# tanmud/video_style_transfer

Hardware: AMD Instinct MI355X
Metric: denoised frames/sec, 16x512x512 clip, 50-step AnimateDiff-XL (higher is better)
Workload: dtype bf16; 1 GPU; BASELINE configs[2]: 16x512x512 clip + UnZipLoRA rank-8 (fused) on all 560 spatial q/k/v/out, 50-step Euler, CFG 7.5 batched (B=2); model=SDXL UNet + AnimateDiff-SDXL motion modules (synthetic weights), global_batch=1, frames=16, resolution=512, parallelism=single, graph=True

## Files before the change

include/vst.h:

```cpp
#ifndef VST_H
#define VST_H
#include <stddef.h>
#ifdef __cplusplus
extern "C" {
#endif

int vst_gemm(const void* A, int lda, const void* A2, int lda2, int K1, const void* W, int ldw, int M, int N, int K,
             const float* bias, const float* row_bias, int row_bias_div, int ld_row_bias, const void* R, int ldr,
             void* C, int ldc, int epilogue, void* stream);
int vst_gemm_ex(const void* A, int lda, const void* A2, int lda2, int K1, const void* W, int ldw, int M, int N, int K,
                const float* bias, const float* row_bias, int row_bias_div, int ld_row_bias, const void* R, int ldr,
                void* C, int ldc, int epilogue, int tile, int splits, void* workspace, size_t ws_bytes,
                void* stream);
size_t vst_gemm_workspace_bytes(int M, int N, int K);

int vst_gemm_lora(const void* x, int ldx, const void* Acat, int ld_acat, int P, int group_n, int group_r,
                  const void* W, int ldw, int M, int N, int K, const float* bias, const void* R, int ldr,
                  void* C, int ldc, void* stream);
int vst_gemm_lora_supported(int M, int N, int K, int P, int group_n, int group_r);
int vst_p8_force_bn(int bn);
int vst_p8_conv(int on);
int vst_p8_persist(int on);

int vst_gemm_temporal_attention(const void* x, int ldx, const void* Wt, int ldw, const float* bias, int M, int K,
                                int nclip, int F, int HW, int heads, int head_dim, float scale, void* O, int ldo,
                                void* stream);
int vst_gemm_temporal_attention_supported(int M, int K, int nclip, int F, int HW, int heads, int head_dim);

int vst_gemm_cross_attention(const void* x, int ldx, const void* Acat, int ld_acat, int P, int group_n, int group_r,
                             const void* W, int ldw, const float* bias, int M, int N, int K, const void* Kt,
                             const void* Vt, int ldkv, int nkv_rows, int Nq, int Nk, int kv_div, float scale, void* O,
                             int ldo, void* stream);
int vst_gemm_cross_attention_supported(int M, int N, int K, int lora, int P, int group_n, int group_r, int Nq,
                                       int Nk);

const char* vst_gemm_kernel_name(int M, int N, int K, int kind, int tile, int splits, size_t ws_bytes);

int vst_conv3x3(const void* x1, int C1, const void* x2, int C2, int nimg, int H, int W, int stride, int upsample,
                const void* Wt, int Cout, const float* bias, const float* row_bias, int row_bias_div, const void* R,
                int ldr, void* out, int ldc, void* stream);
int vst_conv3x3_ex(const void* x1, int C1, const void* x2, int C2, int nimg, int H, int W, int stride, int upsample,
                   const void* Wt, int Cout, const float* bias, const float* row_bias, int row_bias_div,
                   int ld_row_bias, const void* R, int ldr, void* out, int ldc, int tile, int splits, void* workspace,
                   size_t ws_bytes, void* stream);
int vst_conv3x3_colstat(const void* x1, int C1, const void* x2, int C2, int nimg, int H, int W, int stride,
                        int upsample, const void* Wt, int Cout, const float* bias, const float* row_bias,
                        int row_bias_div, int ld_row_bias, const void* R, int ldr, void* out, int ldc,
                        float* colstat, void* stream);

int vst_spatial_attention(const void* q, int ldq, const void* k, const void* v, int ldkv, void* o, int ldo,
                          int nbatch, int heads, int Nq, int Nk, int kv_div, int head_dim, float scale, float* lse,
                          void* stream);
int vst_sa_self(int on);

int vst_temporal_attention(const void* q, const void* k, const void* v, int ldqkv, void* o, int ldo, int nclip,
                           int F, int HW, int heads, int head_dim, float scale, void* stream);

int vst_temporal_attention_windowed(const void* q, const void* k, const void* v, int ldqkv, const float* pos_q,
                                    const float* pos_k, const float* pos_v, int ldpos, void* o, int ldo, int nclip,
                                    int F, int HW, int heads, int head_dim, int L, int S, int weighting, float scale,
                                    void* stream);

int vst_motion_attention_block(const void* x, int ldx, int nclip, int F, int HW, int C, int heads, const float* gamma,
                               const float* beta, float eps, const float* pe, const void* wqkv, int ldw,
                               const float* bqkv, const void* wo, int ldwo, const float* bo, float scale, void* y,
                               int ldy, void* stream);
int vst_motion_attention_block_supported(int C, int F, int HW, int heads);

size_t vst_groupnorm_workspace_bytes(int nsamples, int rows_per_sample, int groups, int C);
int vst_groupnorm(const void* x1, int ld1, int C1, const void* x2, int ld2, int C2, int nsamples,
                  int rows_per_sample, int groups, float eps, const float* gamma, const float* beta, int silu_act,
                  void* y, int ldy, void* workspace, void* stream);
int vst_colstat(const void* x, int ldx, int M, int C, float* cs, void* stream);
int vst_groupnorm_colstat(const void* x1, int ld1, int C1, const float* cs1, const void* x2, int ld2, int C2,
                          const float* cs2, int nsamples, int rows_per_sample, int groups, float eps,
// ... 88 lines not shown
```

video_style_transfer_amd/_lib.py:

```python
from __future__ import annotations

import ctypes
import os

_HERE = os.path.dirname(os.path.abspath(__file__))
LIB_PATH = os.path.join(_HERE, "libvst_hip.so")

_P = ctypes.c_void_p
_I = ctypes.c_int
_F = ctypes.c_float
_S = ctypes.c_size_t
SIGNATURES = {
    "vst_gemm": (_I, [_P, _I, _P, _I, _I, _P, _I, _I, _I, _I, _P, _P, _I, _I, _P, _I, _P, _I, _I, _P]),
    "vst_gemm_ex": (_I, [_P, _I, _P, _I, _I, _P, _I, _I, _I, _I, _P, _P, _I, _I, _P, _I, _P, _I, _I, _I, _I, _P, _S,
                         _P]),
    "vst_gemm_workspace_bytes": (_S, [_I, _I, _I]),
    "vst_gemm_lora": (_I, [_P, _I, _P, _I, _I, _I, _I, _P, _I, _I, _I, _I, _P, _P, _I, _P, _I, _P]),
    "vst_gemm_lora_supported": (_I, [_I, _I, _I, _I, _I, _I]),
    "vst_gemm_cross_attention": (_I, [_P, _I, _P, _I, _I, _I, _I, _P, _I, _P, _I, _I, _I, _P, _P, _I, _I, _I, _I, _I,
                                      _F, _P, _I, _P]),
    "vst_gemm_cross_attention_supported": (_I, [_I, _I, _I, _I, _I, _I, _I, _I, _I]),
    "vst_gemm_temporal_attention": (_I, [_P, _I, _P, _I, _P, _I, _I, _I, _I, _I, _I, _I, _F, _P, _I, _P]),
    "vst_gemm_temporal_attention_supported": (_I, [_I, _I, _I, _I, _I, _I, _I]),
    "vst_gemm_kernel_name": (ctypes.c_char_p, [_I, _I, _I, _I, _I, _I, _S]),
    "vst_conv3x3": (_I, [_P, _I, _P, _I, _I, _I, _I, _I, _I, _P, _I, _P, _P, _I, _P, _I, _P, _I, _P]),
    "vst_conv3x3_ex": (_I, [_P, _I, _P, _I, _I, _I, _I, _I, _I, _P, _I, _P, _P, _I, _I, _P, _I, _P, _I, _I, _I, _P,
                            _S, _P]),
    "vst_spatial_attention": (_I, [_P, _I, _P, _P, _I, _P, _I, _I, _I, _I, _I, _I, _I, _F, _P, _P]),
    "vst_temporal_attention": (_I, [_P, _P, _P, _I, _P, _I, _I, _I, _I, _I, _I, _F, _P]),
    "vst_temporal_attention_windowed": (_I, [_P, _P, _P, _I, _P, _P, _P, _I, _P, _I, _I, _I, _I, _I, _I, _I, _I, _I, _F,
                                             _P]),
    "vst_motion_attention_block": (_I, [_P, _I, _I, _I, _I, _I, _I, _P, _P, _F, _P, _P, _I, _P, _P, _I, _P, _F, _P, _I,
                                        _P]),
    "vst_motion_attention_block_supported": (_I, [_I, _I, _I, _I]),
    "vst_groupnorm_workspace_bytes": (_S, [_I, _I, _I, _I]),
    "vst_groupnorm_frame_chunks": (_I, [_I]),
    "vst_p8_force_bn": (_I, [_I]),
    "vst_p8_conv": (_I, [_I]),
    "vst_p8_persist": (_I, [_I]),
    "vst_sa_self": (_I, [_I]),
    "vst_groupnorm_frame_partials": (_I, [_P, _I, _I, _I, _I, _I, _P, _P]),
    "vst_groupnorm_apply_partials": (_I, [_P, _I, _I, _I, _I, _I, _I, _P, _I, _F, _P, _P, _I, _P, _I, _P, _P]),
    "vst_permute_rows": (_I, [_P, _P, _I, _I, _I, _I, _I, _I, _I, _I, _I, _P]),
    "vst_groupnorm": (_I, [_P, _I, _I, _P, _I, _I, _I, _I, _I, _F, _P, _P, _I, _P, _I, _P, _P]),
    "vst_colstat": (_I, [_P, _I, _I, _I, _P, _P]),
    "vst_groupnorm_colstat": (_I, [_P, _I, _I, _P, _P, _I, _I, _P, _I, _I, _I, _F, _P, _P, _I, _P, _I, _P, _P]),
    "vst_conv3x3_colstat": (_I, [_P, _I, _P, _I, _I, _I, _I, _I, _I, _P, _I, _P, _P, _I, _I, _P, _I, _P, _I, _P,
                                 _P]),
    "vst_layernorm_lora": (_I, [_P, _I, _I, _I, _P, _P, _F, _P, _I, _P, _I, _P, _I, _P]),
    "vst_layernorm": (_I, [_P, _I, _I, _I, _P, _P, _F, _P, _I, _I, _P, _I, _P]),
    "vst_add_row_table": (_I, [_P, _I, _I, _I, _P, _I, _I, _P, _I, _P]),
    "vst_unpack_tokens": (_I, [_P, _I, _I, _I, _I, _P, _P]),
    "vst_timestep_embedding": (_I, [_P, _P, _I, _I, _I, _F, _P, _I, _I, _I, _P]),
    "vst_pack_latents": (_I, [_P, _I, _I, _I, _I, _P, _P, _F, _I, _P, _P]),
    "vst_euler_cfg_step": (_I, [_P, _I, _F, _P, _I, _I, _I, _I, _P, _P, _P]),
    "vst_step_advance": (_I, [_P, _I, _P]),
    "vst_silu": (_I, [_P, _P, _S, _P]),
    "vst_add": (_I, [_P, _P, _P, _S, _P]),
    "vst_quick_gelu": (_I, [_P, _P, _S, _P]),
    "vst_embed_tokens": (_I, [_P, _I, _I, _P, _P, _I, _P, _I, _P]),
    "vst_causal_attention": (_I, [_P, _I, _P, _P, _I, _P, _I, _I, _I, _I, _I, _F, _P]),
    "vst_residual_layernorm": (_I, [_P, _I, _P, _I, _I, _I, _P, _P, _F, _P, _I, _P, _I, _P]),
    "vst_copy2d": (_I, [_P, _I, _P, _I, _I, _I, _P]),
    "vst_transpose": (_I, [_P, _I, _I, _I, _P, _I, _P]),
    "vst_layernorm_bwd_workspace_bytes": (_S, [_I, _I]),
    "vst_layernorm_bwd": (_I, [_P, _I, _P, _I, _I, _I, _P, _F, _P, _I, _P, _P, _P, _P]),
    "vst_geglu_bwd": (_I, [_P, _I, _P, _I, _I, _I, _P, _I, _P]),
    "vst_colsum_workspace_bytes": (_S, [_I, _I]),
    "vst_colsum": (_I, [_P, _I, _I, _I, _P, _P, _P]),
    "vst_groupnorm_bwd_workspace_bytes": (_S, [_I, _I, _I, _I]),
    "vst_groupnorm_bwd": (_I, [_P, _I, _P, _I, _I, _I, _I, _I, _F, _P, _P, _I, _P, _I, _P, _P, _P, _P]),
    "vst_spatial_attention_bwd_workspace_bytes": (_S, [_I, _I, _I, _I]),
    "vst_spatial_attention_bwd": (_I, [_P, _I, _P, _P, _I, _P, _I, _P, _I, _P, _P, _I, _P, _P, _I, _I, _I, _I, _I, _I,
                                       _I, _F, _P, _P]),
    "vst_zero_insert": (_I, [_P, _I, _I, _I, _I, _P, _P]),
    "vst_sumpool2x2": (_I, [_P, _I, _I, _I, _I, _P, _P]),
    "vst_temporal_attention_bwd": (_I, [_P, _P, _P, _I, _P, _I, _P, _P, _P, _I, _I, _I, _I, _I, _I, _F, _P]),
    "vst_conv3x3_down_pad0": (_I, [_P, _I, _I, _I, _I, _P, _I, _P, _P, _I, _P, _S, _P]),
    "vst_gemm_f32out": (_I, [_P, _I, _P, _I, _I, _I, _I, _P, _P]),
    "vst_gemm_tn": (_I, [_P, _I, _P, _I, _I, _I, _I, _P, _I, _P, _S, _P]),
    "vst_gemm_tn_workspace_bytes": (_S, [_I, _I, _I]),
    "vst_softmax_rows": (_I, [_P, _I, _I, _I, _F, _P, _I, _P]),
    "vst_nchw_to_nhwc": (_I, [_P, _I, _I, _I, _F, _P, _I, _P]),
    "vst_nhwc_to_nchw": (_I, [_P, _I, _I, _I, _I, _P, _P]),
    "vst_frames_to_u8": (_I, [_P, _I, _I, _I, _I, _P, _P]),
    "vst_vae_sample": (_I, [_P, _I, _I, _I, _P, _F, _P, _P]),
    "vst_probe_mfma": (_I, [_I, _I, _P, _P]),
    "vst_probe_hbm_read": (_I, [_P, _S, _I, _P, _P]),
    "vst_probe_fetch": (_I, [_I, _P, _I, _I, _I, _P, _P]),
    "vst_probe_mix": (_I, [_I, _I, _P, _I, _I, _I, _P, _P]),
    "vst_version": (ctypes.c_char_p, []),
}
# ... 38 lines not shown
```

video_style_transfer_amd/csrc/gemm_common.h:

```cpp
#pragma once
#include "vst_common.h"

namespace vst {

struct GemmArgs {
  const bf16_t* A1; const bf16_t* A2;
  int lda1, lda2, K1;
  int H, W, C1, C2, OH, OW, stride, up;
  int pad0;
  const bf16_t* Wt; int ldw;
  int M, N, K;
  const float* bias;
  const float* rbias; int rbias_div, ldrb;
  const bf16_t* R; int ldr;
  bf16_t* C; int ldc;
  float* ws;
  int splits;
  int act;
  int persist;
  int group_m;
  int p8_bn;
  int ablate;
  uint32_t a1_bytes, a2_bytes, w_bytes, r_bytes;
  const bf16_t* la;
  int lda_la, la_p, la_gn, la_gr;
  uint32_t la_bytes, wtail_bytes;
  const bf16_t* xa_k;
  const bf16_t* xa_v;
  int xa_ldkv, xa_nk, xa_nq, xa_kvdiv;
  float xa_scale_log2;
  uint32_t xa_kv_bytes;
  int ta_hw, ta_heads, ta_d;
  float ta_scale_log2;
  float* colstat;
};

__device__ __forceinline__ int swz(int row, int chunk) {
  return row * 128 + ((chunk ^ ((row >> 1) & 7)) << 4);
}

}
```

video_style_transfer_amd/csrc/gemm_p8.hip:

```cpp
#include "attn_common.h"
#include "gemm_common.h"
#include "gemm_epilogue.h"

#include <type_traits>

namespace vst {

template <int BN_, int BM_ = 256>
struct P8Cfg {
  static constexpr int BM = BM_, BN = BN_, WAVES_M = 2, WAVES_N = 4, NWAVES = 8, THREADS = 512;
  static constexpr int WM = BM / 2, WN = BN / 4, MI = WM / 16, NJ = WN / 16;
  static constexpr int HALF = WM / 2;
  static constexpr int MQR = HALF / 16;
  static constexpr int NPA = BM / 128;
  static constexpr int RB1 = WN - 32;
  static constexpr int NJ1 = RB1 / 16;
  static constexpr int NPB1 = 4 * RB1 / 64;
  static constexpr int SLOT_A = BM / 2 * 128;
  static constexpr int SLOT_B0 = 128 * 128;
  static constexpr int SLOT_B1 = 4 * RB1 * 128;
  static constexpr int BUF = 2 * SLOT_A + SLOT_B0 + SLOT_B1;
  static constexpr int EPI_BYTES = BM * (BN * 2 + 16);
  static constexpr int LDS = 2 * BUF > EPI_BYTES ? 2 * BUF : EPI_BYTES;
  static constexpr int LORA_OFF = 2 * BUF, V_OFF = 2 * BUF + 5 * 1024, LORA_END = V_OFF + BN * 32;
// ... 425 lines not shown
    float ls = 0.f;
#pragma unroll
    for (int i = 0; i < 4; ++i) {
      s[i] = fast_exp2(s[i] * sl2 - mb);
      ls += s[i];
    }
    ls += __shfl_xor(ls, 16);
    ls += __shfl_xor(ls, 32);
    const float inv = 1.0f / ls;
    const u32x2 pw{pack2bf(s[0], s[1]), pack2bf(s[2], s[3])};
    const s16x4 pb = __builtin_bit_cast(s16x4, pw);
    bf16_t* orow = p.C + (size_t)((b * TF + fr) * p.ta_hw + pg * 16 + pl) * p.ldc + h * TD;
    for (int db = 0; db < DB; ++db) {
      const int d = db * 16 + fr;
      s16x4 va = s16x4{0, 0, 0, 0};
      if (d < TD) {
#pragma unroll
        for (int i = 0; i < 4; ++i) va[i] = *reinterpret_cast<const short*>(R + (4 * g + i) * LROW + (cv + d) * 2);
      }
      const f32x4 o = __builtin_amdgcn_mfma_f32_16x16x16bf16_1k(va, pb, f32x4{0.f, 0.f, 0.f, 0.f}, 0, 0, 0) * inv;
      if (db * 16 + 4 * g < TD)
        *reinterpret_cast<u32x2*>(orow + db * 16 + 4 * g) = u32x2{pack2bf(o[0], o[1]), pack2bf(o[2], o[3])};
    }
  }
}

template <int EPI, int BN, bool LORA = false, int PH = 3, int BM = 256, bool CONV = false, bool PERSIST = false>
__global__ __launch_bounds__(512, 1) void gemm_p8_kernel(GemmArgs p) {
  extern __shared__ __attribute__((aligned(16))) char smem[];
  using Cfg = P8Cfg<BN, BM>;
  static_assert(!CONV || (!LORA && EPI == 0), "conv: plain epilogue");
  static_assert(EPI != 1 || BN == 256, "GEGLU needs 64-column [hidden | gate] blocks");
  static_assert(!LORA || EPI != 1, "in-GEMM LoRA: linear epilogue");
  static_assert(!PERSIST || (!CONV && EPI != 4 && EPI != 5 && PH == 2 && (!LORA || (EPI == 0 && BN == 320))),
                "persistent tiles: plain / GEGLU / GELU, and the in-GEMM LoRA on 128x320 tiles; PH 2");
  static_assert(!(PERSIST && LORA) || Cfg::U_END <= 160 * 1024, "LoRA persistent LDS");
  static_assert(EPI != 5 || (BN == 256 && BM == 256 && !LORA && !CONV), "temporal attention epilogue: 256x256 tiles");
  static_assert(EPI != 4 || (BN == 192 && BM == 256), "cross-attention epilogue: 256 x 192 tiles (3 heads)");
#define VST_P8_VMWAIT_LX(X)                  \
  do {                                       \
    if (LORA && wid < 2) p8_vmwait<(X) + 1>(); \
    else p8_vmwait<(X)>();                   \
  } while (0)
  constexpr bool ONE_A = PERSIST || LORA || EPI == 4 || EPI == 5;
#if defined(VST_P8_DMM)
  constexpr bool DMM = true;
#else
  constexpr bool DMM = false;
#endif
#ifdef VST_P8_LORA_B1E
  constexpr bool B1E = EPI != 1;
#else
  constexpr bool B1E = EPI != 1 && !LORA;
#endif
  constexpr int BUF = Cfg::BUF, RB1 = Cfg::RB1, NJ1 = Cfg::NJ1, NPB1 = Cfg::NPB1, NPA = Cfg::NPA;
  constexpr int HALF = Cfg::HALF, MQR = Cfg::MQR;
  auto slot_off = [](int s_) { return s_ < 2 ? s_ * Cfg::SLOT_A : (s_ == 2 ? 2 * Cfg::SLOT_A : 2 * Cfg::SLOT_A + Cfg::SLOT_B0); };
  const int tid = threadIdx.x, lane = tid & 63;
  const int wid = __builtin_amdgcn_readfirstlane(tid >> 6);
  const int wr = wid >> 2, wc = wid & 3;
  const int fr = lane & 15, fq = lane >> 4;
  const int nbm = (p.M + BM - 1) / BM, nbn = (p.N + BN - 1) / BN;
  const int ntiles = nbm * nbn;
  const int GROUP_M = p.group_m > 0 ? p.group_m : 8;
  auto tile_origin = [&](int t, int& m0, int& n0) {
    const int in_group = GROUP_M * nbn;
    const int gid = t / in_group, first_m = gid * GROUP_M;
    const int gsize = min(nbm - first_m, GROUP_M);
    m0 = (first_m + (t - gid * in_group) % gsize) * BM;
    n0 = ((t - gid * in_group) / gsize) * BN;
  };
  const auto ra1 = make_rsrc(p.A1, p.a1_bytes);
  const auto ra2 = make_rsrc(p.A2 ? p.A2 : p.A1, p.A2 ? p.a2_bytes : 0u);
  const auto rw = make_rsrc(p.Wt, p.w_bytes);
  const int nk = (p.K + 63) / 64;
  const bool ktail = !PERSIST && (p.K & 63) != 0;
  const bool late = wid >= 4;
#ifdef VST_P8_TRACE
  const int abl = p.ablate;
#else
  constexpr int abl = 0;
#endif

  constexpr int NPC = NPB1 > 2 ? NPB1 : 2, PS = 8;
  const int PB = wid;
  uint32_t base1[4][NPC], base2[2][NPC];
  int c8[4][NPC];
  int cv_img[2][NPA], cv_oy[2][NPA], cv_ox[2][NPA];
  int cv_tap[2] = {0, 0}, cv_ci[2] = {0, 0}, cv_ci0[2] = {0, 0};
  bool cv_second[2] = {false, false}, cv_rebase[2] = {true, true};
  const int Ctot = p.C1 + p.C2;
  const auto rl = make_rsrc(LORA ? p.la : p.Wt, LORA ? p.la_bytes : 0u);
  int ub0 = 0, lc8 = 0;
  uint32_t lbase = (uint32_t)kOOB;
  int n0_tile = 0;
  int kofs = 0, nm0 = 0, nn0 = 0;
  bool has_next = false;
  int bias_n0 = 0;
  auto setup_tile = [&](int m0, int n0) {
    n0_tile = n0;
    if constexpr (LORA) {
      ub0 = __builtin_amdgcn_readfirstlane(((n0 / p.la_gn) * p.la_gr) & ~15);
      const int r = 8 * wid + (lane >> 3);
      const int c = (lane & 7) ^ ((r >> 1) & 7);
      lc8 = c * 8;
      lbase = wid < 2 ? (uint32_t)((ub0 + r) * p.lda_la + c * 8) * 2u : (uint32_t)kOOB;
// ... 84 lines not shown
      }
    } else {
      const uint32_t kb = (uint32_t)k0 * 2u;
#pragma unroll
      for (int pc = 0; pc < (s == 3 ? NPB1 : 2); ++pc) {
        const bool kin = live && (!ktail || k0 + c8[s][pc] < p.K);
        p8_dma16(rw, dst + pc * PS * 1024, kin ? (int)(base1[s][pc] + kb) : kOOB);
      }
    }
  };

  auto dma_fast = [&](int s, int kt) {
    if ((abl & 1) && kt > 1) return;
    if ((abl & 64) && s >= 2 && kt > 1) return;
    if ((abl & 128) && s < 2 && kt > 1) return;
    char* dst = smem + ((kofs + kt) & 1) * BUF + slot_off(s) + PB * 1024;
    const int k0 = kt * 64;
    if (CONV && s < 2) {
      conv_dma(s, true, dst);
    } else if (s < 2) {
      const bool second = ONE_A ? false : k0 >= p.K1;
      const uint32_t kb = (uint32_t)(second ? k0 - p.K1 : k0) * 2u;
#pragma unroll
      for (int pc = 0; pc < NPA; ++pc)
        p8_dma16(second ? ra2 : ra1, dst + pc * PS * 1024, (int)((second ? base2[s][pc] : base1[s][pc]) + kb));
    } else {
#pragma unroll
      for (int pc = 0; pc < (s == 3 ? NPB1 : 2); ++pc)
        p8_dma16(rw, dst + pc * PS * 1024, (int)(base1[s][pc] + (uint32_t)k0 * 2u));
    }
  };

  auto dma_lora = [&](int kt, int kend, bool checked, int kbase) {
    if ((abl & 1) && kt > 1) return;
    if constexpr (LORA) {
      if (wid >= 2) return;
      char* dst = smem + Cfg::LORA_OFF + ((kbase + kt) & 1) * 2048 + wid * 1024;
      const int k0 = kt * 64;
      const bool kin = !checked || (kt < kend && k0 + lc8 < p.K);
      p8_dma16(rl, dst, kin ? (int)(lbase + (uint32_t)k0 * 2u) : kOOB);
    }
  };

  f32x4 acc[Cfg::MI][Cfg::NJ];
  f32x4 acc_u[2];
  bf16x8 fl[2];
  bf16x8 fa[MQR][2];
  bf16x8 fb0[2][2], fb1[NJ1 > 2 ? NJ1 : 2][2];
#ifdef VST_P8_TRACE
  for (int i = 0; i < MQR; ++i) for (int h = 0; h < 2; ++h) fa[i][h] = bf16x8{};
  for (int j = 0; j < 2; ++j) for (int h = 0; h < 2; ++h) fb0[j][h] = bf16x8{};
  for (int j = 0; j < NJ1; ++j) for (int h = 0; h < 2; ++h) fb1[j][h] = bf16x8{};
#endif
  auto read_a = [&](int buf, int mq) {
    if (abl & (16 | 128)) return;
    const char* S = smem + buf * BUF + slot_off(mq);
#pragma unroll
    for (int i = 0; i < MQR; ++i) {
      const int ib = LORA ? ((i + wc) & (MQR - 1)) : i;
#pragma unroll
      for (int h = 0; h < 2; ++h) fa[i][h] = *reinterpret_cast<const bf16x8*>(S + p8_off(wr * HALF + ib * 16 + fr, h * 4 + fq));
    }
  };
  auto read_b = [&](int buf, int nq, auto& fb) {
    if (abl & (16 | 64)) return;
    const char* S = smem + buf * BUF + slot_off(2 + nq);
    const int rb = nq == 0 ? 32 : RB1;
#pragma unroll
    for (int j = 0; j < (nq == 0 ? 2 : NJ1); ++j)
#pragma unroll
      for (int h = 0; h < 2; ++h) fb[j][h] = *reinterpret_cast<const bf16x8*>(S + p8_off(wc * rb + j * 16 + fr, h * 4 + fq));
  };
  auto read_l = [&](int buf) {
    if (abl & 16) return;
    if constexpr (LORA) {
      const char* S = smem + Cfg::LORA_OFF + buf * 2048;
#pragma unroll
      for (int h = 0; h < 2; ++h) fl[h] = *reinterpret_cast<const bf16x8*>(S + p8_off(fr, h * 4 + fq));
    }
  };
  auto lora_mfma = [&](f32x4& au, int h) {
    if constexpr (LORA) if (!(abl & 2)) au = __builtin_amdgcn_mfma_f32_16x16x32_bf16(fl[h], fa[0][h], au, 0, 0, 0);
  };
#define VST_P8_QUAD(MQ, NQ, FB)                                                                        \
  if (!(abl & 2)) {                                                                                  \
    _Pragma("unroll") for (int i = 0; i < MQR; ++i) _Pragma("unroll") for (int j = 0; j < ((NQ) == 0 ? 2 : NJ1); ++j) \
        _Pragma("unroll") for (int h = 0; h < 2; ++h) acc[(MQ) * MQR + i][(NQ) * 2 + j] =              \
        __builtin_amdgcn_mfma_f32_16x16x32_bf16(FB[j][h], fa[i][h], acc[(MQ) * MQR + i][(NQ) * 2 + j], 0, 0, 0); \
  }

  auto run_segment = [&](int kb, int ke) {
#pragma unroll
    for (int i = 0; i < Cfg::MI; ++i)
#pragma unroll
      for (int j = 0; j < Cfg::NJ; ++j) acc[i][j] = f32x4{0.f, 0.f, 0.f, 0.f};
    acc_u[0] = acc_u[1] = f32x4{0.f, 0.f, 0.f, 0.f};
    if constexpr (LORA) {
      const int row = wid * 32 + (lane >> 1), n = n0_tile + row;
      const bool ok = row < BN && n < p.N;
      p8_dma16(make_rsrc(p.Wt, p.wtail_bytes), smem + Cfg::V_OFF + wid * 1024,
               ok ? (int)(((uint32_t)n * p.ldw + p.K + ub0 + 8 * (lane & 1)) * 2u) : kOOB);
      if constexpr (BN > 256) {
        const int row2 = 256 + row, n2 = n0_tile + row2;
        if (wid < 2)
          p8_dma16(make_rsrc(p.Wt, p.wtail_bytes), smem + Cfg::V_OFF + (8 + wid) * 1024,
                   row2 < BN && n2 < p.N ? (int)(((uint32_t)n2 * p.ldw + p.K + ub0 + 8 * (lane & 1)) * 2u) : kOOB);
      }
    }
    dma_slot(0, kb, ke, 0); dma_lora(kb, ke, true, 0); dma_slot(2, kb, ke, 0); dma_slot(3, kb, ke, 0);
    dma_slot(1, kb, ke, 0); dma_slot(3, kb + 1, ke, 0); dma_slot(0, kb + 1, ke, 0); dma_lora(kb + 1, ke, true, 0);
    dma_slot(2, kb + 1, ke, 0);
    VST_P8_VMWAIT_LX(2 * NPA + 2 + NPB1);
    p8_barrier();
    VST_P8_STAMP(1)
    read_b(kb & 1, 1, fb1);
    if (late) p8_barrier();
    if (late) __builtin_amdgcn_s_setprio(1);
    auto ktile = [&](int t, auto fast_tag) {
      constexpr bool FAST = decltype(fast_tag)::value;
      auto dma = [&](int s_, int kt) {
        if constexpr (FAST) dma_fast(s_, kt); else dma_slot(s_, kt, ke, 0);
      };
      const int buf = t & 1;
      read_a(buf, 0);
      read_b(buf, 0, fb0);
      read_l(buf);
      if (!(abl & 4)) VST_P8_VMWAIT_LX(NPA + 2 + NPB1);
      dma(1, t + 1);
      p8_barrier();
      lora_mfma(acc_u[0], 0);
      VST_P8_QUAD(0, 0, fb0)
      VST_P8_QUAD(0, 1, fb1)
      lora_mfma(acc_u[0], 1);
      p8_barrier();
      read_a(buf, 1);
      if (!(abl & 4)) VST_P8_VMWAIT_LX(2 * NPA + 2);
      dma(3, t + 2);
      p8_barrier();
      lora_mfma(acc_u[1], 0);
      VST_P8_QUAD(1, 1, fb1)
      lora_mfma(acc_u[1], 1);
      p8_barrier();
      read_b(buf ^ 1, 1, fb1);
      if (!(abl & 4)) p8_vmwait<NPA + NPB1>();
      dma(0, t + 2);
      dma_lora(t + 2, ke, !FAST, 0);
      dma(2, t + 2);
      p8_barrier();
      VST_P8_QUAD(1, 0, fb0)
      p8_barrier();
    };
    int t = kb;
    const int ke_fast = ke - 2 - (ktail ? 1 : 0);
    for (; t < ke_fast; ++t) ktile(t, std::true_type{});
    for (; t < ke; ++t) ktile(t, std::false_type{});
    if (!late) p8_barrier();
    asm volatile("s_waitcnt vmcnt(0) lgkmcnt(0)" ::: "memory");
    p8_barrier();
  };
  auto run_segment2 = [&](int kb, int ke, bool first) {
#pragma unroll
    for (int i = 0; i < Cfg::MI; ++i)
#pragma unroll
      for (int j = 0; j < Cfg::NJ; ++j) acc[i][j] = f32x4{0.f, 0.f, 0.f, 0.f};
    acc_u[0] = acc_u[1] = f32x4{0.f, 0.f, 0.f, 0.f};
    if constexpr (LORA) {
      const int row = wid * 32 + (lane >> 1), n = n0_tile + row;
      const bool ok = row < BN && n < p.N;
      p8_dma16(make_rsrc(p.Wt, p.wtail_bytes), smem + Cfg::V_OFF + wid * 1024,
               ok ? (int)(((uint32_t)n * p.ldw + p.K + ub0 + 8 * (lane & 1)) * 2u) : kOOB);
      if constexpr (BN > 256) {
        const int row2 = 256 + row, n2 = n0_tile + row2;
        if (wid < 2)
          p8_dma16(make_rsrc(p.Wt, p.wtail_bytes), smem + Cfg::V_OFF + (8 + wid) * 1024,
                   row2 < BN && n2 < p.N ? (int)(((uint32_t)n2 * p.ldw + p.K + ub0 + 8 * (lane & 1)) * 2u) : kOOB);
      }
    }
    const bool handed = PERSIST && !first;
    if (!PERSIST || first) {
      dma_slot(0, kb, ke, kofs); dma_lora(kb, ke, true, kofs); dma_slot(2, kb, ke, kofs); dma_slot(3, kb, ke, kofs);
      dma_slot(1, kb, ke, kofs);
      if constexpr (B1E) dma_slot(3, kb + 1, ke, kofs);
      dma_slot(0, kb + 1, ke, kofs); dma_lora(kb + 1, ke, true, kofs); dma_slot(2, kb + 1, ke, kofs);
      VST_P8_VMWAIT_LX(2 * NPA + (B1E ? NPB1 : 0) + 2);
    }
    p8_barrier();
    if constexpr (B1E) read_b((kofs + kb) & 1, 1, fb1);
    VST_P8_STAMP(1)
    if (late) p8_barrier();
    if (late) __builtin_amdgcn_s_setprio(1);
    auto ktile2 = [&](int t, auto fast_tag) {
      constexpr bool FAST = decltype(fast_tag)::value;
      auto dma = [&](int s_, int kt) {
        if constexpr (FAST) {
          dma_fast(s_, kt);
        } else if (PERSIST && kt >= ke && has_next) {
          dma_slot(s_, kt - ke, ke, kofs + ke);
        } else {
          dma_slot(s_, kt, ke, kofs);
        }
      };
      const int buf = (kofs + t) & 1;
      read_a(buf, 0);
      read_b(buf, 0, fb0);
      if constexpr (!B1E) read_b(buf, 1, fb1);
      read_l(buf);
      if (!(abl & 4) && !(handed && (B1E ? t == kb : t <= kb + 1))) VST_P8_VMWAIT_LX(NPA + 2);
      if constexpr (EPI == 1 && PERSIST) {
        if (!FAST && t == ke - 2) {
          const int c = bias_n0 + 4 * lane;
          p8_dma16(make_rsrc(p.bias, p.bias ? (uint32_t)p.N * 4u : 0u), smem + Cfg::EPI_OFF + (wid ? 1024 : 0),
                   wid == 0 && p.bias && c < p.N ? c * 4 : kOOB);
        }
      }
      auto dma_j0 = [&] {
        if (!(handed && t == kb)) {
          if constexpr (!B1E) dma(3, t + 1);
          dma(1, t + 1);
        }
      };
      if constexpr (!DMM) dma_j0();
      asm volatile("s_waitcnt lgkmcnt(0)" ::: "memory");
      p8_barrier();
      lora_mfma(acc_u[0], 0);
      VST_P8_QUAD(0, 0, fb0)
      if constexpr (DMM) dma_j0();
      VST_P8_QUAD(0, 1, fb1)
      lora_mfma(acc_u[0], 1);
      if constexpr (DMM) p8_interleave_dma<(2 + NJ1) * MQR * 2 + (LORA ? 2 : 0), (B1E ? 0 : NPB1) + NPA>();
      p8_barrier();
      read_a(buf, 1);
      if (!(abl & 4) && !(handed && t == kb)) p8_vmwait<NPA>();
      if (PERSIST && !FAST && t == ke - 2 && has_next) setup_tile(nm0, nn0);
      static_assert(!(DMM && LORA && B1E), "DMM + LoRA: the Acat piece must stay younger than B1");
      auto dma_l = [&] {
        if (PERSIST && !FAST && t + 2 >= ke && has_next) dma_lora(t + 2 - ke, ke, true, kofs + ke);
        else dma_lora(t + 2, ke, !FAST, kofs);
      };
      auto dma_j1 = [&] {
        if constexpr (B1E) dma(3, t + 2);
        dma(0, t + 2);
        if constexpr (!DMM) dma_l();
        dma(2, t + 2);
      };
      if constexpr (DMM) dma_l();
      if constexpr (!DMM) dma_j1();
      asm volatile("s_waitcnt lgkmcnt(0)" ::: "memory");
      p8_barrier();
      lora_mfma(acc_u[1], 0);
      VST_P8_QUAD(1, 1, fb1)
      if constexpr (DMM) dma_j1();
      if constexpr (B1E) {
        if (t + 1 < ke) read_b(buf ^ 1, 1, fb1);
      }
      VST_P8_QUAD(1, 0, fb0)
      lora_mfma(acc_u[1], 1);
      if constexpr (DMM) p8_interleave_dma<(2 + NJ1) * MQR * 2 + (LORA ? 2 : 0), (B1E ? NPB1 : 0) + NPA + 2>();
      if constexpr (B1E) asm volatile("s_waitcnt lgkmcnt(0)" ::: "memory");
      p8_barrier();
    };
    int t = kb;
    const int ke_fast = ke - 2 - (ktail ? 1 : 0);
    for (; t < ke_fast; ++t) ktile2(t, std::true_type{});
    for (; t < ke; ++t) ktile2(t, std::false_type{});
    if (!late) p8_barrier();
    if constexpr (PERSIST) {
      asm volatile("s_waitcnt lgkmcnt(0)" ::: "memory");
    } else {
      asm volatile("s_waitcnt vmcnt(0) lgkmcnt(0)" ::: "memory");
    }
    p8_barrier();
  };
#undef VST_P8_QUAD
#undef VST_P8_VMWAIT_LX

  auto lora_post = [&](char* U) {
#pragma unroll
    for (int q = 0; q < 2; ++q) {
      u32x2 v;
      v[0] = pack2bf(acc_u[q][0], acc_u[q][1]);
      v[1] = pack2bf(acc_u[q][2], acc_u[q][3]);
      if (wc < MQR) *reinterpret_cast<u32x2*>(U + (wr * Cfg::WM + q * HALF + wc * 16 + fr) * 32 + fq * 8) = v;
    }
    asm volatile("s_waitcnt lgkmcnt(0)" ::: "memory");
    __builtin_amdgcn_s_barrier();
    const bf16x8 zero8 = {};
    bf16x8 fv[Cfg::NJ];
#pragma unroll
    for (int j = 0; j < Cfg::NJ; ++j) {
      const bf16x8 v = *reinterpret_cast<const bf16x8*>(smem + Cfg::V_OFF + (wc * Cfg::WN + j * 16 + fr) * 32 + (fq & 1) * 16);
      fv[j] = fq < 2 ? v : zero8;
    }
#pragma unroll
    for (int i = 0; i < Cfg::MI; ++i) {
      bf16x8 fu = *reinterpret_cast<const bf16x8*>(U + (wr * Cfg::WM + p8_acc_row<Cfg, true>(i, wc) + fr) * 32 + (fq & 1) * 16);
      fu = fq < 2 ? fu : zero8;
#pragma unroll
      for (int j = 0; j < Cfg::NJ; ++j) acc[i][j] = __builtin_amdgcn_mfma_f32_16x16x32_bf16(fv[j], fu, acc[i][j], 0, 0, 0);
    }
    asm volatile("s_waitcnt lgkmcnt(0)" ::: "memory");
    __builtin_amdgcn_s_barrier();
  };
  int m0, n0;
  VST_P8_STAMP(0)
  constexpr int EREG = LORA ? Cfg::EPI_REGION_L : Cfg::EPI_REGION;
  if constexpr (PERSIST) {
    const int xcd = blockIdx.x & 7, loc = blockIdx.x >> 3, per = gridDim.x >> 3;
    const int q = ntiles >> 3, r = ntiles & 7;
    const int beg = xcd < r ? xcd * (q + 1) : r * (q + 1) + (xcd - r) * q;
    const int cnt = q + (xcd < r ? 1 : 0);
    if (loc >= cnt) return;
    int j = loc;
    tile_origin(beg + j, m0, n0);
    setup_tile(m0, n0);
    bool first = true;
    while (true) {
      const int jn = j + per;
// ... 20 lines not shown
          if constexpr (!B1E) dma_slot(3, 1, nk, kofs + nk);
          dma_slot(1, 1, nk, kofs + nk);
        }
      });
#endif
      if (has_next) {
        p8_vmwait<p8_epi_stores<Cfg, EPI, EREG>()>();
        asm volatile("s_waitcnt lgkmcnt(0)" ::: "memory");
      } else {
        asm volatile("s_waitcnt vmcnt(0) lgkmcnt(0)" ::: "memory");
      }
      p8_barrier();
      if (!has_next) return;
      j = jn;
      m0 = nm0;
      n0 = nn0;
      kofs += nk;
      first = false;
    }
  }
  tile_origin(xcd_remap(blockIdx.x, ntiles), m0, n0);
  setup_tile(m0, n0);
  if constexpr (PH == 2) run_segment2(0, nk, true);
  else run_segment(0, nk);
  VST_P8_STAMP(2)
  if constexpr (LORA) lora_post(smem);
#ifdef VST_ABL_NOEPI
  {
    float sink = 0.f;
    for (int i = 0; i < Cfg::MI; ++i)
      for (int jj = 0; jj < Cfg::NJ; ++jj) sink += acc[i][jj][0];
    if (sink == 1234.5f) p.C[0] = 0;
  }
#else
  if constexpr (EPI == 4) xattn_epilogue<Cfg, LORA>(p, smem, m0, n0, acc, wr, wc);
  else if constexpr (EPI == 5) tattn_epilogue<Cfg>(p, smem, m0, n0, acc, wr, wc);
  else tile_epilogue<Cfg, EPI, LORA, CONV>(p, smem, m0, n0, acc, wr, wc);
#endif
#ifdef VST_P8_TRACE
  asm volatile("s_waitcnt vmcnt(0)" ::: "memory");
  __syncthreads();
#endif
  VST_P8_STAMP(3)
}

static int p8_ph_env() {
  static const int v = [] {
    const char* e = getenv("VST_P8_PH");
    return e ? atoi(e) : 2;
  }();
  return v;
}

template <int EPI, int BN, bool LORA, int PH, int BM, bool CONV = false>
static int launch_p8_ph(const GemmArgs& a, hipStream_t s) {
  static bool attr = false;
  using Cfg = P8Cfg<BN, BM>;
  constexpr int lds = EPI == 4 ? 160 * 1024 : (LORA ? Cfg::LDS_LORA : Cfg::LDS);
  if (!attr) {
    (void)hipFuncSetAttribute((const void*)gemm_p8_kernel<EPI, BN, LORA, PH, BM, CONV>,
                              hipFuncAttributeMaxDynamicSharedMemorySize, lds);
    attr = true;
  }
  const int nwg = ((a.M + BM - 1) / BM) * ((a.N + BN - 1) / BN);
  hipLaunchKernelGGL((gemm_p8_kernel<EPI, BN, LORA, PH, BM, CONV>), dim3(nwg), dim3(512), lds, s, a);
  return hipGetLastError() == hipSuccess ? VST_OK : VST_ERR_LAUNCH;
}

static int g_p8_persist = -1;
static int p8_persist_env() {
  if (g_p8_persist < 0) {
    const char* e = getenv("VST_P8_PERSIST");
    g_p8_persist = e ? atoi(e) : 1;
  }
  return g_p8_persist;
}
static int p8_cus() {
  static const int v = [] {
    int dev = 0, n = 0;
    if (hipGetDevice(&dev) != hipSuccess ||
        hipDeviceGetAttribute(&n, hipDeviceAttributeMultiprocessorCount, dev) != hipSuccess || n < 8)
      n = 256;
    return n & ~7;
  }();
  return v;
}

bool p8_persist_applies(int M, int N, int K, int epi, int bn) {
  if (!p8_persist_env() || p8_ph_env() != 2 || (epi != 0 && epi != 1 && epi != 3)) return false;
  const int bm = bn == 320 ? 128 : 256;
  const long tiles = (long)((M + bm - 1) / bm) * ((N + bn - 1) / bn);
  return tiles >= 2L * p8_cus() && K >= 128 && (K & 63) == 0 && (N % (epi == 1 ? 16 : 8)) == 0;
}

template <int EPI, int BN, int BM, bool LORA = false>
static int launch_p8_persist(const GemmArgs& a, hipStream_t s) {
  static bool attr = false;
  if (!attr) {
    (void)hipFuncSetAttribute((const void*)gemm_p8_kernel<EPI, BN, LORA, 2, BM, false, true>,
                              hipFuncAttributeMaxDynamicSharedMemorySize, 160 * 1024);
    attr = true;
  }
  const int ntiles = ((a.M + BM - 1) / BM) * ((a.N + BN - 1) / BN);
  const int grid = ntiles < p8_cus() ? (ntiles & ~7) : p8_cus();
  if (grid < 8) return VST_ERR_ARG;
  hipLaunchKernelGGL((gemm_p8_kernel<EPI, BN, LORA, 2, BM, false, true>), dim3(grid), dim3(512), 160 * 1024, s, a);
  return hipGetLastError() == hipSuccess ? VST_OK : VST_ERR_LAUNCH;
}

static int p8_lora_persist_env() {
  static const int v = [] {
    const char* e = getenv("VST_P8_LORA_PERSIST");
    return e ? atoi(e) : 1;
  }();
  return v;
}
bool p8_lora_persist_on() { return p8_persist_env() && p8_ph_env() == 2 && p8_lora_persist_env(); }

template <int EPI, int BN, bool LORA = false>
static int launch_p8_epi(const GemmArgs& a, hipStream_t s) {
  constexpr int BM = BN == 320 ? 128 : 256;
  if constexpr (!LORA && EPI != 4 && EPI != 5)
    if (!a.A2 && (size_t)a.M * a.ldc * 2 < 0x7fff0000u && p8_persist_applies(a.M, a.N, a.K, EPI, BN))
      return launch_p8_persist<EPI, BN, BM>(a, s);
  if constexpr (LORA && EPI == 0 && BN == 320)
    if (p8_lora_persist_on() && !a.A2 && (size_t)a.M * a.ldc * 2 < 0x7fff0000u &&
        p8_persist_applies(a.M, a.N, a.K, EPI, BN))
      return launch_p8_persist<EPI, BN, BM, true>(a, s);
  return p8_ph_env() == 2 ? launch_p8_ph<EPI, BN, LORA, 2, BM>(a, s) : launch_p8_ph<EPI, BN, LORA, 3, BM>(a, s);
}

int launch_gemm_p8_lora(const GemmArgs& a, int bn, hipStream_t s) {
  if (!a.la) return VST_ERR_ARG;
  if (bn == 320) return launch_p8_epi<0, 320, true>(a, s);
  return bn == 192 ? launch_p8_epi<0, 192, true>(a, s) : launch_p8_epi<0, 256, true>(a, s);
}

int launch_gemm_p8_tattn(const GemmArgs& a, hipStream_t s) {
  if (a.ta_hw <= 0 || (a.ta_hw & 15) || a.A2 || (a.M & 255)) return VST_ERR_ARG;
  return launch_p8_epi<5, 256>(a, s);
}

int launch_gemm_p8_xattn(const GemmArgs& a, hipStream_t s) {
  if (!a.xa_k || !a.xa_v) return VST_ERR_ARG;
  return a.la ? launch_p8_epi<4, 192, true>(a, s) : launch_p8_epi<4, 192, false>(a, s);
}

int launch_gemm_p8_conv(const GemmArgs& a, int bn, hipStream_t s) {
  if ((a.C1 & 63) || (a.C2 & 63) || a.K != 9 * (a.C1 + a.C2)) return VST_ERR_ARG;
  const bool ph2 = p8_ph_env() == 2;
  switch (bn) {
    case 256: return ph2 ? launch_p8_ph<0, 256, false, 2, 256, true>(a, s) : launch_p8_ph<0, 256, false, 3, 256, true>(a, s);
    case 192: return ph2 ? launch_p8_ph<0, 192, false, 2, 256, true>(a, s) : launch_p8_ph<0, 192, false, 3, 256, true>(a, s);
    case 320: return ph2 ? launch_p8_ph<0, 320, false, 2, 128, true>(a, s) : launch_p8_ph<0, 320, false, 3, 128, true>(a, s);
    default: return VST_ERR_ARG;
  }
}

int launch_gemm_p8(const GemmArgs& a, int epi, int bn, hipStream_t s) {
  if (a.A2 && (a.K1 & 63)) return VST_ERR_ARG;
  if (bn == 192 || bn == 320) {
    switch (epi) {
      case 0: return bn == 192 ? launch_p8_epi<0, 192>(a, s) : launch_p8_epi<0, 320>(a, s);
      case 3: return bn == 192 ? launch_p8_epi<3, 192>(a, s) : launch_p8_epi<3, 320>(a, s);
      default: return VST_ERR_ARG;
    }
  }
  if (bn != 256) return VST_ERR_ARG;
  switch (epi) {
    case 0: return launch_p8_epi<0, 256>(a, s);
    case 1: return launch_p8_epi<1, 256>(a, s);
    case 3: return launch_p8_epi<3, 256>(a, s);
    default: return VST_ERR_ARG;
  }
}

}

extern "C" int vst_p8_persist(int on) {
  const int prev = vst::p8_persist_env() ? 1 : 0;
  vst::g_p8_persist = on ? 1 : 0;
  return prev;
}

#ifdef VST_P8_TRACE
extern "C" int vst_p8_trace_read(void* host_dst, int n_wg) {
  if (n_wg > 8192) n_wg = 8192;
  return hipMemcpyFromSymbol(host_dst, HIP_SYMBOL(vst::vst_p8_trace_buf), (size_t)n_wg * 64, 0,
                             hipMemcpyDeviceToHost) == hipSuccess ? 0 : 2;
}
#endif
```

video_style_transfer_amd/kernels.py:

```python
from __future__ import annotations

import os
import weakref

import torch

from . import _lib

BF16 = torch.bfloat16
F32 = torch.float32


def _stream():
    return torch.cuda.current_stream().cuda_stream


_PROF = None


def profile_launches(active: bool):
    global _PROF
    _PROF = [] if active else None


# ... 196 lines not shown
        ws = _workspace(x.device)
        _lib.call("vst_gemm_ex", _p(x), _ld(x), _p(x2), 0 if x2 is None else _ld(x2), K1, _p(w), _ld(w), M, N, K,
                  _p(bias), _p(row_bias), row_bias_div,
                  0 if row_bias is None else (_ld(row_bias) if row_bias.dim() == 2 else N), _p(residual),
                  0 if residual is None else _ld(residual), _p(out), _ld(out), 1 if geglu else (2 if act else 0),
                  GEMM_POLICY["tile"], _splits(), _p(ws), _WS_BYTES, _stream())
    return out


def linear_tn(a: torch.Tensor, b: torch.Tensor, out: torch.Tensor | None = None) -> torch.Tensor:
    _dev(a, BF16, "a")
    _dev(b, BF16, "b")
    M, N = a.shape
    if b.shape[0] != M:
        raise _lib.VstError(f"linear_tn: a {tuple(a.shape)} and b {tuple(b.shape)} differ in tokens")
    K = b.shape[1]
    if out is None:
        out = torch.empty((N, K), dtype=BF16, device=a.device)
    _out(out, (N, K), BF16, "out", "linear_tn")
    wsb = int(_lib.load().vst_gemm_tn_workspace_bytes(M, N, K))
    ws = torch.empty(max(wsb // 4, 1), dtype=F32, device=a.device) if wsb else None
    with _Rec("gemm_tn", 2.0 * M * N * K, 2.0 * (M * N + M * K + N * K), lambda: "gemm_tn", (N, K, M)):
        _lib.call("vst_gemm_tn", _p(a), _ld(a), _p(b), _ld(b), M, N, K, _p(out), _ld(out), _p(ws), wsb, _stream())
    return out


_LORA_BN = {}


class p8_conv:

    def __init__(self, on=True):
        self.on = int(bool(on))

    def __enter__(self):
        self.prev = int(_lib.load().vst_p8_conv(self.on))
        return self

    def __exit__(self, *a):
        _lib.load().vst_p8_conv(self.prev)


class p8_persist:

    def __init__(self, on=True):
        self.on = int(bool(on))

    def __enter__(self):
        self.prev = int(_lib.load().vst_p8_persist(self.on))
        return self

    def __exit__(self, *a):
        _lib.load().vst_p8_persist(self.prev)


class sa_self:

    def __init__(self, on=True):
        self.on = int(bool(on))

    def __enter__(self):
        self.prev = int(_lib.load().vst_sa_self(self.on))
        return self

    def __exit__(self, *a):
        _lib.load().vst_sa_self(self.prev)


class p8_tile_width:

    def __init__(self, bn):
        self.bn = int(bn)

    def __enter__(self):
        self.prev = int(_lib.load().vst_p8_force_bn(self.bn))
        _LORA_BN.clear()
        _XATTN_OK.clear()
        return self

    def __exit__(self, *a):
        _lib.load().vst_p8_force_bn(self.prev)
        _LORA_BN.clear()
        _XATTN_OK.clear()


def gemm_lora_tile(M, N, K, P, group_n, group_r):
    key = (M, N, K, P, group_n, group_r)
    bn = _LORA_BN.get(key)
    if bn is None:
        bn = _LORA_BN[key] = int(_lib.load().vst_gemm_lora_supported(M, N, K, P, group_n, group_r))
    return bn


def linear_lora(x: torch.Tensor, w: torch.Tensor, a: torch.Tensor, group_n: int, group_r: int,
                bias: torch.Tensor | None = None, *, residual: torch.Tensor | None = None,
                out: torch.Tensor | None = None, r_alg: int | None = None) -> torch.Tensor:
    _dev(x, BF16, "x")
    _dev(w, BF16, "w")
    _dev(a, BF16, "a")
    M, K = x.shape
    N = w.shape[0]
    P = a.shape[0]
    if a.shape[1] != K or w.shape[1] != K + P:
        raise _lib.VstError(f"linear_lora: x {tuple(x.shape)} a {tuple(a.shape)} w {tuple(w.shape)}")
    if out is None:
        out = torch.empty((M, N), dtype=BF16, device=x.device)
# ... 832 lines not shown
```

Measured before the change: 4.975 frames/s.

## Interleave next-tile LDS fragment reads with MFMAs in p8 GEMM late path

Adds a 'late refill' schedule to the p8 GEMM k-loop. LDS fragment reads for the next half-tile and next k-tile are issued one at a time between MFMAs, using sched_group_barrier hints, instead of in a batch before the MFMA block. The goal is to hide LDS read latency behind matrix math. In the default build it is enabled only for the conv GEMM with BN=320 on the late-barrier path, and it is switchable by env var or API. It raises register pressure and scheduling complexity, and it adds one more kernel template specialisation.

Measured after the change: 4.998 frames/s (median of 4 runs). Within noise of the previous version (+0.5%).

```diff
diff --git a/include/vst.h b/include/vst.h
--- a/include/vst.h
+++ b/include/vst.h
@@ -21,6 +21,8 @@
 int vst_p8_force_bn(int bn);
 int vst_p8_conv(int on);
 int vst_p8_persist(int on);
+
+int vst_p8_late_refill(int on);
 
 int vst_gemm_temporal_attention(const void* x, int ldx, const void* Wt, int ldw, const float* bias, int M, int K,
                                 int nclip, int F, int HW, int heads, int head_dim, float scale, void* O, int ldo,
diff --git a/video_style_transfer_amd/_lib.py b/video_style_transfer_amd/_lib.py
--- a/video_style_transfer_amd/_lib.py
+++ b/video_style_transfer_amd/_lib.py
@@ -38,6 +38,7 @@
     "vst_p8_force_bn": (_I, [_I]),
     "vst_p8_conv": (_I, [_I]),
     "vst_p8_persist": (_I, [_I]),
+    "vst_p8_late_refill": (_I, [_I]),
     "vst_sa_self": (_I, [_I]),
     "vst_groupnorm_frame_partials": (_I, [_P, _I, _I, _I, _I, _I, _P, _P]),
     "vst_groupnorm_apply_partials": (_I, [_P, _I, _I, _I, _I, _I, _I, _P, _I, _F, _P, _P, _I, _P, _I, _P, _P]),
diff --git a/video_style_transfer_amd/csrc/gemm_common.h b/video_style_transfer_amd/csrc/gemm_common.h
--- a/video_style_transfer_amd/csrc/gemm_common.h
+++ b/video_style_transfer_amd/csrc/gemm_common.h
@@ -21,6 +21,7 @@
   int group_m;
   int p8_bn;
   int ablate;
+  int late_refill;
   uint32_t a1_bytes, a2_bytes, w_bytes, r_bytes;
   const bf16_t* la;
   int lda_la, la_p, la_gn, la_gr;
diff --git a/video_style_transfer_amd/csrc/gemm_p8.hip b/video_style_transfer_amd/csrc/gemm_p8.hip
--- a/video_style_transfer_amd/csrc/gemm_p8.hip
+++ b/video_style_transfer_amd/csrc/gemm_p8.hip
@@ -501,6 +501,11 @@
   constexpr bool B1E = EPI != 1;
 #else
   constexpr bool B1E = EPI != 1 && !LORA;
+#endif
+#ifdef VST_P8_LR_BUILD
+  constexpr bool LRC = PH == 2 && !(EPI == 0 && BN == 256 && !LORA && (PERSIST || CONV));
+#else
+  constexpr bool LRC = PH == 2 && CONV && BN == 320;
 #endif
   constexpr int BUF = Cfg::BUF, RB1 = Cfg::RB1, NJ1 = Cfg::NJ1, NPB1 = Cfg::NPB1, NPA = Cfg::NPA;
   constexpr int HALF = Cfg::HALF, MQR = Cfg::MQR;
@@ -691,32 +696,38 @@
   for (int j = 0; j < 2; ++j) for (int h = 0; h < 2; ++h) fb0[j][h] = bf16x8{};
   for (int j = 0; j < NJ1; ++j) for (int h = 0; h < 2; ++h) fb1[j][h] = bf16x8{};
 #endif
+  auto read_a1 = [&](const char* S, int i, int h) {
+    if (abl & (16 | 128)) return;
+    const int ib = LORA ? ((i + wc) & (MQR - 1)) : i;
+    fa[i][h] = *reinterpret_cast<const bf16x8*>(S + p8_off(wr * HALF + ib * 16 + fr, h * 4 + fq));
+  };
+  auto read_b1 = [&](const char* S, int rb, auto& fb, int j, int h) {
+    if (abl & (16 | 64)) return;
+    fb[j][h] = *reinterpret_cast<const bf16x8*>(S + p8_off(wc * rb + j * 16 + fr, h * 4 + fq));
+  };
+  auto read_l1 = [&](int buf, int h) {
+    if (abl & 16) return;
+    if constexpr (LORA)
+      fl[h] = *reinterpret_cast<const bf16x8*>(smem + Cfg::LORA_OFF + buf * 2048 + p8_off(fr, h * 4 + fq));
+  };
   auto read_a = [&](int buf, int mq) {
-    if (abl & (16 | 128)) return;
     const char* S = smem + buf * BUF + slot_off(mq);
 #pragma unroll
-    for (int i = 0; i < MQR; ++i) {
-      const int ib = LORA ? ((i + wc) & (MQR - 1)) : i;
-#pragma unroll
-      for (int h = 0; h < 2; ++h) fa[i][h] = *reinterpret_cast<const bf16x8*>(S + p8_off(wr * HALF + ib * 16 + fr, h * 4 + fq));
-    }
+    for (int i = 0; i < MQR; ++i)
+#pragma unroll
+      for (int h = 0; h < 2; ++h) read_a1(S, i, h);
   };
   auto read_b = [&](int buf, int nq, auto& fb) {
-    if (abl & (16 | 64)) return;
     const char* S = smem + buf * BUF + slot_off(2 + nq);
     const int rb = nq == 0 ? 32 : RB1;
 #pragma unroll
     for (int j = 0; j < (nq == 0 ? 2 : NJ1); ++j)
 #pragma unroll
-      for (int h = 0; h < 2; ++h) fb[j][h] = *reinterpret_cast<const bf16x8*>(S + p8_off(wc * rb + j * 16 + fr, h * 4 + fq));
+      for (int h = 0; h < 2; ++h) read_b1(S, rb, fb, j, h);
   };
   auto read_l = [&](int buf) {
-    if (abl & 16) return;
-    if constexpr (LORA) {
-      const char* S = smem + Cfg::LORA_OFF + buf * 2048;
-#pragma unroll
-      for (int h = 0; h < 2; ++h) fl[h] = *reinterpret_cast<const bf16x8*>(S + p8_off(fr, h * 4 + fq));
-    }
+#pragma unroll
+    for (int h = 0; h < 2; ++h) read_l1(buf, h);
   };
   auto lora_mfma = [&](f32x4& au, int h) {
     if constexpr (LORA) if (!(abl & 2)) au = __builtin_amdgcn_mfma_f32_16x16x32_bf16(fl[h], fa[0][h], au, 0, 0, 0);
@@ -727,6 +738,11 @@
         _Pragma("unroll") for (int h = 0; h < 2; ++h) acc[(MQ) * MQR + i][(NQ) * 2 + j] =              \
         __builtin_amdgcn_mfma_f32_16x16x32_bf16(FB[j][h], fa[i][h], acc[(MQ) * MQR + i][(NQ) * 2 + j], 0, 0, 0); \
   }
+  auto mfma1 = [&](int mq, int i, int nq, auto& fb, int j, int h) {
+    if (!(abl & 2))
+      acc[mq * MQR + i][nq * 2 + j] =
+          __builtin_amdgcn_mfma_f32_16x16x32_bf16(fb[j][h], fa[i][h], acc[mq * MQR + i][nq * 2 + j], 0, 0, 0);
+  };
 
   auto run_segment = [&](int kb, int ke) {
 #pragma unroll
@@ -828,8 +844,11 @@
     VST_P8_STAMP(1)
     if (late) p8_barrier();
     if (late) __builtin_amdgcn_s_setprio(1);
-    auto ktile2 = [&](int t, auto fast_tag) {
+    auto ktile2 = [&](int t, auto fast_tag, auto lr_tag) {
       constexpr bool FAST = decltype(fast_tag)::value;
+      constexpr bool LR = decltype(lr_tag)::value;
+      auto sg_mfma = [] { __builtin_amdgcn_sched_group_barrier(0x008, 1, 0); };
+      auto sg_read = [] { __builtin_amdgcn_sched_group_barrier(0x100, 1, 0); };
       auto dma = [&](int s_, int kt) {
         if constexpr (FAST) {
           dma_fast(s_, kt);
@@ -840,10 +859,12 @@
         }
       };
       const int buf = (kofs + t) & 1;
-      read_a(buf, 0);
-      read_b(buf, 0, fb0);
-      if constexpr (!B1E) read_b(buf, 1, fb1);
-      read_l(buf);
+      if constexpr (!LR) {
+        read_a(buf, 0);
+        read_b(buf, 0, fb0);
+        if constexpr (!B1E) read_b(buf, 1, fb1);
+        read_l(buf);
+      }
       if (!(abl & 4) && !(handed && (B1E ? t == kb : t <= kb + 1))) VST_P8_VMWAIT_LX(NPA + 2);
       if constexpr (EPI == 1 && PERSIST) {
         if (!FAST && t == ke - 2) {
@@ -861,14 +882,50 @@
       if constexpr (!DMM) dma_j0();
       asm volatile("s_waitcnt lgkmcnt(0)" ::: "memory");
       p8_barrier();
-      lora_mfma(acc_u[0], 0);
-      VST_P8_QUAD(0, 0, fb0)
-      if constexpr (DMM) dma_j0();
-      VST_P8_QUAD(0, 1, fb1)
-      lora_mfma(acc_u[0], 1);
-      if constexpr (DMM) p8_interleave_dma<(2 + NJ1) * MQR * 2 + (LORA ? 2 : 0), (B1E ? 0 : NPB1) + NPA>();
+      if constexpr (LR) {
+        const char* S1 = smem + buf * BUF + slot_off(1);
+        int nr = 0, avail = 0;
+        auto pop = [&] {
+          if (nr < avail) {
+            read_a1(S1, nr >> 1, nr & 1);
+            if constexpr (!DMM) sg_read();
+            ++nr;
+          }
+        };
+        if constexpr (DMM) dma_j0();
+#pragma unroll
+        for (int i = 0; i < MQR; ++i) {
+#pragma unroll
+          for (int j = 0; j < 2 + NJ1; ++j)
+#pragma unroll
+            for (int h = 0; h < 2; ++h) {
+              if (j < 2) mfma1(0, i, 0, fb0, j, h);
+              else mfma1(0, i, 1, fb1, j - 2, h);
+              if constexpr (!DMM) sg_mfma();
+              pop();
+            }
+          if (i == 0) {
+#pragma unroll
+            for (int h = 0; h < 2; ++h) {
+              lora_mfma(acc_u[0], h);
+              if constexpr (LORA && !DMM) sg_mfma();
+            }
+          }
+          avail += 2;
+        }
+        pop();
+        pop();
+        if constexpr (DMM) p8_interleave_dma<(2 + NJ1) * MQR * 2 + (LORA ? 2 : 0), (B1E ? 0 : NPB1) + NPA>();
+      } else {
+        lora_mfma(acc_u[0], 0);
+        VST_P8_QUAD(0, 0, fb0)
+        if constexpr (DMM) dma_j0();
+        VST_P8_QUAD(0, 1, fb1)
+        lora_mfma(acc_u[0], 1);
+        if constexpr (DMM) p8_interleave_dma<(2 + NJ1) * MQR * 2 + (LORA ? 2 : 0), (B1E ? 0 : NPB1) + NPA>();
+      }
       p8_barrier();
-      read_a(buf, 1);
+      if constexpr (!LR) read_a(buf, 1);
       if (!(abl & 4) && !(handed && t == kb)) p8_vmwait<NPA>();
       if (PERSIST && !FAST && t == ke - 2 && has_next) setup_tile(nm0, nn0);
       static_assert(!(DMM && LORA && B1E), "DMM + LoRA: the Acat piece must stay younger than B1");
@@ -886,22 +943,82 @@
       if constexpr (!DMM) dma_j1();
       asm volatile("s_waitcnt lgkmcnt(0)" ::: "memory");
       p8_barrier();
-      lora_mfma(acc_u[1], 0);
-      VST_P8_QUAD(1, 1, fb1)
-      if constexpr (DMM) dma_j1();
-      if constexpr (B1E) {
-        if (t + 1 < ke) read_b(buf ^ 1, 1, fb1);
-      }
-      VST_P8_QUAD(1, 0, fb0)
-      lora_mfma(acc_u[1], 1);
-      if constexpr (DMM) p8_interleave_dma<(2 + NJ1) * MQR * 2 + (LORA ? 2 : 0), (B1E ? NPB1 : 0) + NPA + 2>();
-      if constexpr (B1E) asm volatile("s_waitcnt lgkmcnt(0)" ::: "memory");
+      if constexpr (LR) {
+        constexpr int LF = LORA ? 2 : 0, RA = LF + 2 * (MQR - 1), RB1_ = RA + 2 * NJ1, RB0_ = RB1_ + 4;
+        const char* SA = smem + (buf ^ 1) * BUF + slot_off(0);
+        const char* SB0 = smem + (buf ^ 1) * BUF + slot_off(2);
+        const char* SB1 = smem + (buf ^ 1) * BUF + slot_off(3);
+        int nr = 0, avail = 0;
+        auto pop = [&] {
+          if (nr < avail) {
+            if (nr < 2) read_a1(SA, 0, nr);
+            else if (nr < 2 + LF) read_l1(buf ^ 1, nr - 2);
+            else if (nr < RA) read_a1(SA, (nr - LF) >> 1, (nr - LF) & 1);
+            else if (nr < RB1_) read_b1(SB1, RB1, fb1, (nr - RA) >> 1, (nr - RA) & 1);
+            else if (nr < RB0_) read_b1(SB0, 32, fb0, (nr - RB1_) >> 1, (nr - RB1_) & 1);
+            else read_a1(SA, MQR - 1, nr - RB0_);
+            if constexpr (!DMM) sg_read();
+            ++nr;
+          }
+        };
+        if constexpr (DMM) dma_j1();
+#pragma unroll
+        for (int i = 0; i < MQR; ++i) {
+#pragma unroll
+          for (int j = 0; j < NJ1 + 2; ++j)
+#pragma unroll
+            for (int h = 0; h < 2; ++h) {
+              if (j < NJ1) mfma1(1, i, 1, fb1, j, h);
+              else mfma1(1, i, 0, fb0, j - NJ1, h);
+              if constexpr (!DMM) sg_mfma();
+              if (i == MQR - 1) ++avail;
+              pop();
+            }
+          if (i == 0) {
+#pragma unroll
+            for (int h = 0; h < 2; ++h) {
+              lora_mfma(acc_u[1], h);
+              if constexpr (LORA && !DMM) sg_mfma();
+            }
+            avail += LF;
+          }
+          avail += 2;
+        }
+#pragma unroll
+        for (int r = 0; r < 4 + LF; ++r) pop();
+        if constexpr (DMM) p8_interleave_dma<(2 + NJ1) * MQR * 2 + (LORA ? 2 : 0), (B1E ? NPB1 : 0) + NPA + 2>();
+      } else {
+        lora_mfma(acc_u[1], 0);
+        VST_P8_QUAD(1, 1, fb1)
+        if constexpr (DMM) dma_j1();
+        if constexpr (B1E) {
+          if (t + 1 < ke) read_b(buf ^ 1, 1, fb1);
+        }
+        VST_P8_QUAD(1, 0, fb0)
+        lora_mfma(acc_u[1], 1);
+        if constexpr (DMM) p8_interleave_dma<(2 + NJ1) * MQR * 2 + (LORA ? 2 : 0), (B1E ? NPB1 : 0) + NPA + 2>();
+        if constexpr (B1E) asm volatile("s_waitcnt lgkmcnt(0)" ::: "memory");
+      }
       p8_barrier();
     };
     int t = kb;
     const int ke_fast = ke - 2 - (ktail ? 1 : 0);
-    for (; t < ke_fast; ++t) ktile2(t, std::true_type{});
-    for (; t < ke; ++t) ktile2(t, std::false_type{});
+    bool lr = false;
+    if constexpr (LRC) lr = late && p.late_refill;
+    if (lr) {
+      {
+        const int buf = (kofs + kb) & 1;
+        read_a(buf, 0);
+        read_b(buf, 0, fb0);
+        if constexpr (!B1E) read_b(buf, 1, fb1);
+        read_l(buf);
+      }
+      for (; t < ke_fast; ++t) ktile2(t, std::true_type{}, std::bool_constant<LRC>{});
+      for (; t < ke; ++t) ktile2(t, std::false_type{}, std::bool_constant<LRC>{});
+    } else {
+      for (; t < ke_fast; ++t) ktile2(t, std::true_type{}, std::false_type{});
+      for (; t < ke; ++t) ktile2(t, std::false_type{}, std::false_type{});
+    }
     if (!late) p8_barrier();
     if constexpr (PERSIST) {
       asm volatile("s_waitcnt lgkmcnt(0)" ::: "memory");
@@ -1028,8 +1145,19 @@
   return v;
 }
 
+static int g_p8_late_refill = -1;
+static int p8_late_refill_env() {
+  if (g_p8_late_refill < 0) {
+    const char* e = getenv("VST_P8_LATE_REFILL");
+    g_p8_late_refill = e ? (atoi(e) ? 1 : 0) : 1;
+  }
+  return g_p8_late_refill;
+}
+
 template <int EPI, int BN, bool LORA, int PH, int BM, bool CONV = false>
-static int launch_p8_ph(const GemmArgs& a, hipStream_t s) {
+static int launch_p8_ph(const GemmArgs& a_, hipStream_t s) {
+  GemmArgs a = a_;
+  a.late_refill = PH == 2 ? p8_late_refill_env() : 0;
   static bool attr = false;
   using Cfg = P8Cfg<BN, BM>;
   constexpr int lds = EPI == 4 ? 160 * 1024 : (LORA ? Cfg::LDS_LORA : Cfg::LDS);
@@ -1070,7 +1198,9 @@
 }
 
 template <int EPI, int BN, int BM, bool LORA = false>
-static int launch_p8_persist(const GemmArgs& a, hipStream_t s) {
+static int launch_p8_persist(const GemmArgs& a_, hipStream_t s) {
+  GemmArgs a = a_;
+  a.late_refill = p8_late_refill_env();
   static bool attr = false;
   if (!attr) {
     (void)hipFuncSetAttribute((const void*)gemm_p8_kernel<EPI, BN, LORA, 2, BM, false, true>,
@@ -1159,6 +1289,12 @@
   return prev;
 }
 
+extern "C" int vst_p8_late_refill(int on) {
+  const int prev = vst::p8_late_refill_env() ? 1 : 0;
+  vst::g_p8_late_refill = on ? 1 : 0;
+  return prev;
+}
+
 #ifdef VST_P8_TRACE
 extern "C" int vst_p8_trace_read(void* host_dst, int n_wg) {
   if (n_wg > 8192) n_wg = 8192;
diff --git a/video_style_transfer_amd/kernels.py b/video_style_transfer_amd/kernels.py
--- a/video_style_transfer_amd/kernels.py
+++ b/video_style_transfer_amd/kernels.py
@@ -272,6 +272,19 @@
 
     def __exit__(self, *a):
         _lib.load().vst_p8_persist(self.prev)
+
+
+class p8_late_refill:
+
+    def __init__(self, on=True):
+        self.on = int(bool(on))
+
+    def __enter__(self):
+        self.prev = int(_lib.load().vst_p8_late_refill(self.on))
+        return self
+
+    def __exit__(self, *a):
+        _lib.load().vst_p8_late_refill(self.prev)
 
 
 class sa_self:
```
